# astro-turing/Integrating-diagenetic-equations-using-Python

Measured on AMD Instinct MI355X. Metric: grid-point-steps/sec (5 fields, fp64), higher is better.
Workload: dtype f64

## Files before the change

include/marl_hip.h:

```cpp
#ifndef MARL_HIP_H
#define MARL_HIP_H

#include "marl_params.h"

#ifdef __cplusplus
extern "C" {
#endif

typedef struct marl_ctx marl_ctx;

#define MARL_LAYOUT_FIELD_MAJOR 0
#define MARL_LAYOUT_TILED 1

int marl_ctx_create(const marl_params* params, int64_t n_instances, int64_t N, int device, marl_ctx** out);
int marl_ctx_set_params(marl_ctx* ctx, const marl_params* params, int64_t n_instances);

void marl_ctx_destroy(marl_ctx* ctx);
const char* marl_last_error(const marl_ctx* ctx);
int marl_set_stream(marl_ctx* ctx, void* hip_stream);
int marl_synchronize(marl_ctx* ctx);
int marl_set_option(marl_ctx* ctx, const char* name, int64_t value);
int marl_get_constants(const marl_ctx* ctx, int64_t inst, double out[19]);
int64_t marl_state_doubles(const marl_ctx* ctx, int layout);

int marl_rhs(marl_ctx* ctx, double t, const double* y, double* dydt);
int marl_rhs_dev(marl_ctx* ctx, double t, const double* y_dev, double* dydt_dev, int layout);

int marl_events(marl_ctx* ctx, const double* y, double* out);
int marl_events_dev(marl_ctx* ctx, const double* y_dev, int layout, double* out);

int marl_convert_layout_dev(marl_ctx* ctx, const double* src_dev, double* dst_dev, int src_layout, int dst_layout);

int marl_debug_math(marl_ctx* ctx, int op, const double* x_dev, double* y_dev, int64_t n, double e);

int marl_integrate_rk4(marl_ctx* ctx, double* y, double dt, int64_t nsteps);
int marl_integrate_rk4_dev(marl_ctx* ctx, double* y_dev, int layout, double dt, int64_t nsteps);
int marl_sweep_rk4_dev(marl_ctx* ctx, double* y_dev, const double* dt, int64_t nsteps);

// ... 50 lines not shown
```

integrating-diagenetic-equations-using-python_amd/_abi.py:

```python
import ctypes as C
import os

_HERE = os.path.dirname(os.path.abspath(__file__))
LIB_PATH = os.environ.get("MARL_HIP_LIBRARY") or os.path.join(_HERE, "csrc", "libmarl_hip.so")



def lab_options():
    out = []
    for item in os.environ.get("MARL_HIP_OPTIONS", "").split(","):
        if item.strip():
            name, _, value = item.partition("=")
            out.append((name.strip(), int(value)))
    return out


def library_fingerprint():
    import hashlib
    with open(LIB_PATH, "rb") as f:
        return LIB_PATH, hashlib.sha256(f.read()).hexdigest()[:16]


NFIELDS = 5
NEVENTS = 7
# ... 24 lines not shown

_P = C.c_void_p
_D = C.c_double
_I = C.c_int
_L = C.c_int64
PROTOTYPES = {
    "marl_ctx_create": (_I, [C.POINTER(MarlParams), _L, _L, _I, C.POINTER(_P)]),
    "marl_ctx_set_params": (_I, [_P, C.POINTER(MarlParams), _L]),
    "marl_ctx_destroy": (None, [_P]),
    "marl_last_error": (C.c_char_p, [_P]),
    "marl_set_stream": (_I, [_P, _P]),
    "marl_synchronize": (_I, [_P]),
    "marl_set_option": (_I, [_P, C.c_char_p, _L]),
    "marl_get_constants": (_I, [_P, _L, C.POINTER(_D)]),
    "marl_state_doubles": (_L, [_P, _I]),
    "marl_rhs": (_I, [_P, _D, _P, _P]),
    "marl_rhs_dev": (_I, [_P, _D, _P, _P, _I]),
    "marl_events": (_I, [_P, _P, _P]),
    "marl_events_dev": (_I, [_P, _P, _I, _P]),
    "marl_convert_layout_dev": (_I, [_P, _P, _P, _I, _I]),
    "marl_debug_math": (_I, [_P, _I, _P, _P, _L, _D]),
    "marl_integrate_rk4": (_I, [_P, _P, _D, _L]),
    "marl_integrate_rk4_dev": (_I, [_P, _P, _I, _D, _L]),
    "marl_sweep_rk4_dev": (_I, [_P, _P, _P, _L]),
    "marl_integrate_rk45": (_I, [_P, _P, _D, _D, _D, _D, _D, _P, _L, _P, _P, _L, _L, C.POINTER(MarlStats)]),
    "marl_integrate_rk45_dev": (_I, [_P, _P, _I, _D, _D, _D, _D, _D, _L, C.POINTER(MarlStats)]),
    "marl_sweep_rk45_dev": (_I, [_P, _P, _D, _D, _D, _D, _D, _L, C.POINTER(MarlStats)]),
    "marl_sweep_rk45_eval_dev": (_I, [_P, _P, _D, _D, _D, _D, _D, _L, _P, _L, _P, _P, C.POINTER(MarlStats)]),
    "marl_sweep_rk45_events_dev": (_I, [_P, _P, _D, _D, _D, _D, _D, _L, _P, _L, _P, _P, _P, _L, C.POINTER(MarlStats)]),
    "marl_integrate_radau": (_I, [_P, _P, _D, _D, _D, _D, _D, _P, _P, _L, _P, _P, _L, _L, C.POINTER(MarlStats)]),
# ... 53 lines not shown
```

integrating-diagenetic-equations-using-python_amd/csrc/marl_api.hip:

```cpp
#include <hip/hip_runtime.h>

#include <dlfcn.h>

#include <cmath>
#include <cstdarg>
#include <cstdio>
#include <cstring>
#include <string>
#include <vector>

#include "../../include/marl_hip.h"
#include "marl_kernels.h"
#include "marl_radau.h"
#include "marl_radau_cr.h"
#include "marl_radau_batch.h"
#include "marl_radau_wg.h"
#include "marl_bdf.h"
#include "marl_bdf_wg.h"

using namespace marl;

static_assert(MARL_NFIELDS == NF, "field count");
constexpr int64_t kChainMax = 8;
static thread_local std::string g_create_error;
// ... 48 lines not shown
    int64_t dd_max_attempts = 0;
    void* rccl_lib = nullptr;
    void* rccl_comm = nullptr;
    int (*rccl_allgather)(const void*, void*, size_t, int, void*, hipStream_t) = nullptr;
    int (*rccl_destroy)(void*) = nullptr;
    double* rd_arena = nullptr;
    size_t rd_cap = 0;
    double* rd_host = nullptr;
    double* zc_h = nullptr;
    double* zc_d = nullptr;
    bool zc_on = false;
    int64_t rk4_variant = -1, sweep_variant = -1, host_layout = LAYOUT_TILED, poll = 64;
    int64_t rk4_stream = 1;
    int64_t rk4_small = 1;
    int64_t rk4_chain = 1;
    int64_t rk4_stream_third = 1;
    double* stream_c = nullptr;
    size_t stream_c_cap = 0;
    int64_t implicit_zero_copy = 1;
    int64_t radau_fused_solve = 3;
    int64_t radau_solver = 0;
    int64_t radau_cr = -1;
    int64_t radau_cr_min_n = 2048;
    int64_t radau_cr_small = 3;
    int64_t radau_cr_small_min_n = 205;
    int64_t bdf_solve_wg = 1;
    int64_t radau_cr_tail = 1;
    int64_t radau_sweep_wg = 3;
    std::string err;
};
// ... 172 lines not shown

int marl_ctx_set_params(marl_ctx* ctx, const marl_params* params, int64_t n_instances)
{
    if (!ctx || !params) return ctx ? fail(ctx, -1, "marl_ctx_set_params: invalid argument") : -1;
    if (n_instances != ctx->batch) return fail(ctx, -1, "marl_ctx_set_params: the context holds %lld instance(s)", (long long)ctx->batch);
    if (ctx->halo > 0) return fail(ctx, -1, "marl_ctx_set_params: not for slab contexts");
    for (int64_t b = 0; b < n_instances; b++) {
        if (!(params[b].length > 0)) return fail(ctx, -1, "marl_ctx_set_params: instance %lld: length must be > 0", (long long)b);
        if ((params[b].dPhi_variable != 0) != (params[0].dPhi_variable != 0))
            return fail(ctx, -1, "marl_ctx_set_params: dPhi_variable must be the same for every instance of a sweep");
    }
    HIP_OK(ctx, hipSetDevice(ctx->device));
    HIP_OK(ctx, hipStreamSynchronize(ctx->stream));
    ctx->params.assign(params, params + n_instances);
    const int no_reuse = ctx->hconsts[0].hot.no_reuse;
    for (int64_t b = 0; b < n_instances; b++) {
        derive_consts(params[b], ctx->N, ctx->hconsts[b], &ctx->extra[4 * b]);
        ctx->hconsts[b].hot.no_reuse = no_reuse;
    }
    ctx->var_dphi = params[0].dPhi_variable != 0;
    HIP_OK(ctx, hipMemcpyAsync(ctx->dconsts, ctx->hconsts.data(), sizeof(DevConsts) * n_instances, hipMemcpyHostToDevice, ctx->stream));
    HIP_OK(ctx, hipStreamSynchronize(ctx->stream));
    return 0;
}

void marl_ctx_destroy(marl_ctx* ctx)
{
    if (!ctx) return;
    (void)hipSetDevice(ctx->device);
    (void)hipStreamSynchronize(ctx->stream);
    for (int i = 0; i < 4; i++)
        if (ctx->buf[i]) (void)hipFree(ctx->buf[i]);
    if (ctx->part) (void)hipFree(ctx->part);
    if (ctx->stream_c) (void)hipFree(ctx->stream_c);
    if (ctx->sq) (void)hipFree(ctx->sq);
    if (ctx->sq_sticky) (void)hipFree(ctx->sq_sticky);
    if (ctx->sq_host) (void)hipHostFree(ctx->sq_host);
    if (ctx->rs) (void)hipFree(ctx->rs);
    if (ctx->rs_grec) (void)hipFree(ctx->rs_grec);
    if (ctx->rs_host) (void)hipHostFree(ctx->rs_host);
    if (ctx->rec) (void)hipFree(ctx->rec);
    if (ctx->dctrl) (void)hipFree(ctx->dctrl);
    if (ctx->ddt) (void)hipFree(ctx->ddt);
    if (ctx->dconsts) (void)hipFree(ctx->dconsts);
    if (ctx->hctrl) (void)hipHostFree(ctx->hctrl);
    if (ctx->hrec) (void)hipHostFree(ctx->hrec);
    if (ctx->hdt) (void)hipHostFree(ctx->hdt);
    if (ctx->sw_teval) (void)hipFree(ctx->sw_teval);
    if (ctx->sw_ndone) (void)hipFree(ctx->sw_ndone);
// ... 60 lines not shown
    else if (n == "radau_cr_min_n") ctx->radau_cr_min_n = std::max<int64_t>(value, 4);
    else if (n == "radau_cr_small") ctx->radau_cr_small = value < 0 ? 0 : std::min<int64_t>(value, radau::CR_WG_MAX_LEVELS);
    else if (n == "radau_cr_small_min_n") ctx->radau_cr_small_min_n = std::max<int64_t>(value, 32);
    else if (n == "radau_cr_tail") ctx->radau_cr_tail = value ? 1 : 0;
    else if (n == "bdf_solve_wg") ctx->bdf_solve_wg = value ? 1 : 0;
    else if (n == "radau_fused_solve") ctx->radau_fused_solve = value < 0 ? 0 : (value > 3 ? 3 : value);
    else if (n == "radau_sweep_wg") ctx->radau_sweep_wg = value < 0 ? 0 : (value > 3 ? 3 : value);
    else if (n == "implicit_zero_copy") ctx->implicit_zero_copy = value ? 1 : 0;
    else if (n == "rk4_stream") ctx->rk4_stream = value < 0 ? 0 : (value > 2 ? 2 : value);
    else if (n == "rk45_stream") ctx->rk45_stream = value < 0 ? 0 : (value > 2 ? 2 : value);
    else if (n == "dd_stream") ctx->dd_stream = value < 0 ? 0 : (value > 2 ? 2 : value);
    else if (n == "rk45_stream_attempts") ctx->rk45_stream_attempts = value < 1 ? 1 : std::min<int64_t>(value, 1 << 20);
    else if (n == "rk4_small") ctx->rk4_small = value ? 1 : 0;
    else if (n == "rk4_chain") ctx->rk4_chain = value < 0 ? 0 : std::min<int64_t>(value, kChainMax);
    else if (n == "rk4_stream_third") ctx->rk4_stream_third = value ? 1 : 0;
    else if (n == "rk4_stream_test_raise") ctx->sq_test_raise = value != 0;
    else if (n == "rk4_stream_max_items") ctx->sq_max_items = value > 0 ? std::min<int64_t>(value, 0x7fffffff) : 0x7fffffff;
    else if (n == "no_reuse") {
        for (auto& c : ctx->hconsts) c.hot.no_reuse = value ? 1 : 0;
        HIP_OK(ctx, hipSetDevice(ctx->device));
        HIP_OK(ctx, hipStreamSynchronize(ctx->stream));
        HIP_OK(ctx, hipMemcpy(ctx->dconsts, ctx->hconsts.data(), sizeof(DevConsts) * ctx->hconsts.size(), hipMemcpyHostToDevice));
    }
    else return fail(ctx, -1, "marl_set_option: unknown option '%s'", name);
    return 0;
}

int marl_get_constants(const marl_ctx* ctx, int64_t inst, double out[19])
{
    if (!ctx || inst < 0 || inst >= ctx->batch || !out) return -1;
    const DevConsts& d = ctx->hconsts[inst];
    const HotConsts& c = d.hot;
    const double* x = &ctx->extra[4 * inst];
    const double v[19] = {x[0], c.nu1, c.nu2, c.KRat, c.dCa, c.dCO3, c.delta, c.Da, c.lambda_, x[1], x[2], c.rhorat,
                          c.presum, x[3], c.dPhi, PECLET_MIN, PECLET_MAX, (double)d.mask_lo, (double)d.mask_hi};
    memcpy(out, v, sizeof v);
    return 0;
}

int64_t marl_state_doubles(const marl_ctx* ctx, int layout) { return ctx ? state_doubles(ctx->slab.n_buf, layout) : -1; }

}

#ifndef MARL_LAB
static inline int64_t inst_stride(const marl_ctx* ctx, int layout) { return state_doubles(ctx->slab.n_buf, layout); }

static int launch_rhs(marl_ctx* ctx, const double* y, double* dydt, int layout, int64_t nstates = 0)
{
    const dim3 grid((unsigned)((ctx->slab.n_buf + 255) / 256), (unsigned)(nstates > 0 ? nstates : ctx->batch));
    const int64_t stride = inst_stride(ctx, layout);
    const int cs = nstates > 0 ? 0 : 1;
    if (ctx->var_dphi) {
        if (layout == LAYOUT_TILED)
            hipLaunchKernelGGL((rhs_kernel<LAYOUT_TILED, true>), grid, dim3(256), 0, ctx->stream, y, dydt, ctx->dconsts, ctx->slab, stride, cs);
        else
// ... 57 lines not shown
{
    constexpr int V = 256 - 8 * NSTEPS;
    const int64_t n = ctx->slab.out_hi - ctx->slab.out_lo;
    const dim3 grid((unsigned)((n + V - 1) / V));
    if (layout == LAYOUT_TILED)
        hipLaunchKernelGGL((rk4_fused_kernel<256, LAYOUT_TILED, NSTEPS, VD>), grid, dim3(256), 0, ctx->stream, yin, yout, ctx->dconsts, ctx->slab, dt);
    else
        hipLaunchKernelGGL((rk4_fused_kernel<256, LAYOUT_FIELD_MAJOR, NSTEPS, VD>), grid, dim3(256), 0, ctx->stream, yin, yout, ctx->dconsts, ctx->slab, dt);
}

constexpr int kVdRk4Depth = 4;

extern "C" int marl_small_rk4_16(int tiled, unsigned grid, hipStream_t stream, const double* yin, double* yout, const void* consts, const int64_t slab5[5],
                                 double dt);

static int launch_rk4(marl_ctx* ctx, int nsteps, const double* yin, double* yout, int layout, double dt)
{
    switch (nsteps) {
        case 1: if (ctx->var_dphi) launch_rk4_t<1, true>(ctx, yin, yout, layout, dt); else launch_rk4_t<1>(ctx, yin, yout, layout, dt); break;
        case 2: launch_rk4_t<2>(ctx, yin, yout, layout, dt); break;
        case 4: if (ctx->var_dphi) launch_rk4_t<4, true>(ctx, yin, yout, layout, dt); else launch_rk4_t<4>(ctx, yin, yout, layout, dt); break;
        case 8: launch_rk4_t<8>(ctx, yin, yout, layout, dt); break;
        case 16: {
            const int64_t n = ctx->slab.out_hi - ctx->slab.out_lo, V = 256 - 8 * 16, tiles = (n + V - 1) / V;
            if (!ctx->cus) {
                hipDeviceProp_t prop;
                HIP_OK(ctx, hipGetDeviceProperties(&prop, ctx->device));
                ctx->cus = prop.multiProcessorCount;
            }
            if (ctx->rk4_small && tiles <= 2 * (int64_t)ctx->cus) {
                const int64_t slab5[5] = {ctx->slab.n_buf, ctx->slab.goff, ctx->slab.ld, ctx->slab.out_lo, ctx->slab.out_hi};
                const int e = marl_small_rk4_16(layout == LAYOUT_TILED, (unsigned)tiles, ctx->stream, yin, yout, ctx->dconsts, slab5, dt);
// ... 99 lines not shown
    while (levels > 0) {
        const int64_t cap = (ctx->sq_max_items / tiles) & ~(int64_t)1;
        const int64_t lv = std::min<int64_t>(levels, std::max<int64_t>(cap, 2));
        const unsigned blocks = (unsigned)std::min<int64_t>(lv * tiles, (4 * 256 / MARL_LAB_STREAM_BLK) * (int64_t)ctx->cus);
        double* c = nullptr;
        if (ctx->rk4_stream_third && levels == lv && (lv & 1) && lv >= 3) {
            const size_t need = (size_t)state_doubles(ctx->slab.n_buf, layout);
            if (ctx->stream_c_cap < need) {
                if (ctx->stream_c) HIP_OK(ctx, hipFree(ctx->stream_c));
                ctx->stream_c = nullptr; ctx->stream_c_cap = 0;
                HIP_OK(ctx, hipMalloc((void**)&ctx->stream_c, need * sizeof(double)));
                ctx->stream_c_cap = need;
            }
            c = ctx->stream_c;
        }
        if (K >= 2) {
            if (layout == LAYOUT_TILED) launch_chain_t<LAYOUT_TILED>(ctx, a, b, dt, (unsigned)lv, shape, blocks, c);
            else launch_chain_t<LAYOUT_FIELD_MAJOR>(ctx, a, b, dt, (unsigned)lv, shape, blocks, c);
        } else switch (per) {
            case 1: if (ctx->var_dphi) launch_stream_t<1, true>(ctx, a, b, layout, dt, (unsigned)lv, (unsigned)tiles, blocks, c);
                    else launch_stream_t<1>(ctx, a, b, layout, dt, (unsigned)lv, (unsigned)tiles, blocks, c);
                    break;
            case 2: launch_stream_t<2>(ctx, a, b, layout, dt, (unsigned)lv, (unsigned)tiles, blocks, c); break;
            case 4: if (ctx->var_dphi) launch_stream_t<4, true>(ctx, a, b, layout, dt, (unsigned)lv, (unsigned)tiles, blocks, c);
                    else launch_stream_t<4>(ctx, a, b, layout, dt, (unsigned)lv, (unsigned)tiles, blocks, c);
                    break;
            case 8: launch_stream_t<8>(ctx, a, b, layout, dt, (unsigned)lv, (unsigned)tiles, blocks, c); break;
            case 16: launch_stream_t<16>(ctx, a, b, layout, dt, (unsigned)lv, (unsigned)tiles, blocks, c); break;
            default: return fail(ctx, -1, "rk4 stream: %d steps per level not instantiated", per);
        }
// ... 2187 lines not shown
```

integrating-diagenetic-equations-using-python_amd/csrc/marl_kernels.h:

```cpp
#pragma once
#include <type_traits>

#include "marl_math.h"
#include "marl_brent.h"

namespace marl {

enum : int { LAYOUT_FIELD_MAJOR = 0, LAYOUT_TILED = 1 };

template <int LAYOUT>
__device__ __forceinline__ int64_t at(int f, int64_t i, int64_t ld)
{
    if constexpr (LAYOUT == LAYOUT_FIELD_MAJOR)
        return (int64_t)f * ld + i;
    else
        return (i >> 6) * (int64_t)(NF * 64) + f * 64 + (i & 63);
}

struct Slab {
    int64_t n_buf;
    int64_t goff;
    int64_t ld;
    int64_t out_lo;
    int64_t out_hi;
// ... 5 lines not shown
__device__ __forceinline__ double mon_min(double a, double b) { return FINITE ? __builtin_fmin(a, b) : nanmin(a, b); }
template <bool FINITE = false>
__device__ __forceinline__ double mon_max(double a, double b) { return FINITE ? __builtin_fmax(a, b) : nanmax(a, b); }


#ifdef MARL_LAB_PHASE_CLOCK
__device__ unsigned long long marl_lab_phase[8];
#define MARL_PHASE_MARK(k) do { const unsigned long long t_ = __builtin_amdgcn_s_memtime(); ph_acc[k] += t_ - ph_last; ph_last = t_; } while (0)
#else
#define MARL_PHASE_MARK(k) do { } while (0)
#endif

#define MARL_ONCE _Pragma("unroll") for (int once_ = 0; once_ < 1; once_++)
#define MARL_FIELDS _Pragma("unroll") for (int f = 0; f < NF; f++)

template <int BLK, bool REUSE = true, bool VD = false, int SEAM = 0>
struct StencilBlock {
    static constexpr int EDGE_DOUBLES = 2 * NF * BLK;
    static constexpr bool CACHE_LDS = PC_LDS_SLOTS > 0;
    static constexpr bool CACHE = REUSE && (EDGE_DOUBLES + TABLE_DOUBLES + PC_LDS_SLOTS * BLK) * 8 <= 60 * 1024;
    static constexpr int CACHE_DOUBLES = CACHE ? PC_LDS_SLOTS * BLK : 0;
    static constexpr int LDS_DOUBLES = EDGE_DOUBLES + TABLE_DOUBLES + CACHE_DOUBLES;

    double* lds;
    Tables T;
    HotConsts K;
    const DevConsts* C;
    int tid;
    int parity;
    unsigned masks;
    static constexpr bool EDGE_ONCE = CACHE;
    unsigned edge_cells;
    __device__ __forceinline__ bool edge_wave() const
    {
        if constexpr (EDGE_ONCE) return edge_cells & 1u;
        else return __builtin_amdgcn_ballot_w64(is_edge() != 0) != 0;
    }
    __device__ __forceinline__ unsigned is_first() const { return masks & 1u; }
    __device__ __forceinline__ unsigned is_last() const { return (masks >> 8) & 1u; }
    __device__ __forceinline__ unsigned in_zone() const { return (masks >> 16) & 1u; }
    __device__ __forceinline__ unsigned is_edge() const { return masks & 0x101u; }
    PointCache<(CACHE && CACHE_LDS) ? BLK : 0> cache;
    bool reuse_live = false;
    static constexpr int SEAM_STRIDE = 16, SEAM_READS = 0x10000, SEAM_WAVE0 = 0x20000, SEAM_WAVEW = 0x40000;
    static_assert(SEAM < BLK, "the recording lane is a lane of the window");
    double* seam = nullptr;
// ... 36 lines not shown
#pragma unroll
        for (int f = 0; f < NF; f++) e[f * BLK + tid] = ys[f];
        if constexpr (SEAM > 0) {
            if (seam_pos & SEAM_WAVEW) {
                int tw = tid;
                asm volatile("" : "+v"(tw));
                if (tw == SEAM) {
                    double* rec = seam + (seam_pos & 0xffff);
#pragma unroll
                    for (int f = 0; f < NF; f++) rec[f] = ys[f];
                }
            }
        }
        MARL_PHASE_MARK(0);
        PointLocal pl;
        MARL_ONCE point_local<CACHE ? MODE : TR_PLAIN, (CACHE && CACHE_LDS) ? BLK : 0, VD>(ys, in_zone(), K, C, T, pl, aux, cache, reuse_live);
        MARL_PHASE_MARK(1);
        __syncthreads();
        MARL_PHASE_MARK(2);
        const int tl = tid > 0 ? tid - 1 : 0;
        const int tr = tid < BLK - 1 ? tid + 1 : BLK - 1;
        double left[NF], right[NF];
#pragma unroll
        for (int f = 0; f < NF; f++) left[f] = e[f * BLK + tl];
        if constexpr (SEAM > 0) {
            if ((seam_pos & (SEAM_WAVE0 | SEAM_READS)) == (SEAM_WAVE0 | SEAM_READS)) {
                int t0 = tid;
                asm volatile("" : "+v"(t0));
                if (t0 == 0) {
                    const double* prev = seam + ((seam_pos & 0xffff) ^ 8);
#pragma unroll
// ... 283 lines not shown

#ifndef MARL_LAB_RK4_WAVES_MIN
#define MARL_LAB_RK4_WAVES_MIN 4
#define MARL_LAB_RK4_WAVES_MAX 8
#endif
template <int BLK, int LAYOUT, int NSTEPS, bool VD = false>
__global__ void __launch_bounds__(BLK) __attribute__((amdgpu_waves_per_eu(MARL_LAB_RK4_WAVES_MIN, MARL_LAB_RK4_WAVES_MAX))) rk4_fused_kernel(const double* __restrict__ yin, double* __restrict__ yout,
                                                        const DevConsts* __restrict__ consts, Slab S, double dt)
{
#ifdef MARL_LAB_CLOCK
    const unsigned long long lab_t0 = __builtin_amdgcn_s_memtime(), lab_r0 = __builtin_amdgcn_s_memrealtime();
#endif
    constexpr int H = 4 * NSTEPS;
    constexpr int V = BLK - 2 * H;
    static_assert(V > 0, "window too small for the fused halo");
    using SB = StencilBlock<BLK, true, VD>;
    __shared__ double lds[SB::LDS_DOUBLES];
    const DevConsts& C = consts[0];

    const int64_t w0 = S.out_lo + (int64_t)blockIdx.x * V - H;
    const int64_t l = w0 + (int64_t)threadIdx.x;
    double y[NF];
    load_cells<LAYOUT>(yin, l, S, C, y);
    SB sb(lds, l + S.goff, consts);
    rk4_advance<NSTEPS>(sb, y, dt);

    const int wi = threadIdx.x;
    MARL_ONCE if (wi >= H && wi < BLK - H && l >= S.out_lo && l < S.out_hi) {
#pragma unroll
        for (int f = 0; f < NF; f++) yout[at<LAYOUT>(f, l, S.ld)] = y[f];
    }
#ifdef MARL_LAB_PHASE_CLOCK
    sb.phase_flush();
#endif
#ifdef MARL_LAB_CLOCK
    if (threadIdx.x == 0 && blockIdx.x < 16384) {
        marl_lab_clock[3 * blockIdx.x] = __builtin_amdgcn_s_memtime() - lab_t0;
        marl_lab_clock[3 * blockIdx.x + 1] = __builtin_amdgcn_s_memrealtime() - lab_r0;
        marl_lab_clock[3 * blockIdx.x + 2] = lab_r0;
    }
#endif
}

constexpr unsigned STREAM_SPIN_LIMIT = 1u << 19;

template <int BLK, int LAYOUT, int NSTEPS, bool VD = false>
__global__ void __launch_bounds__(BLK) __attribute__((amdgpu_waves_per_eu(4, 8)))
rk4_stream_kernel(double* bufA, double* bufB, const DevConsts* __restrict__ consts, Slab S, double dt, unsigned levels, unsigned tiles,
                  unsigned* queue, unsigned* done, unsigned* sticky, unsigned item_base, unsigned level_base, double* bufC = nullptr)
{
    constexpr int H = 4 * NSTEPS;
    constexpr int V = BLK - 2 * H;
    using SB = StencilBlock<BLK, true, VD>;
    __shared__ double lds[SB::LDS_DOUBLES];
    __shared__ unsigned s_item, s_abort;
    const DevConsts& C = consts[0];
    SB sb(lds, 0, consts);
    const unsigned total = levels * tiles;

#ifdef MARL_LAB_BROKEN_STREAM_LATCH
    if (threadIdx.x == 0) {
        s_item = __hip_atomic_fetch_add(&queue[0], 1u, __ATOMIC_RELAXED, __HIP_MEMORY_SCOPE_AGENT) - item_base;
        s_abort = 0;
    }
    while (true) {
        __syncthreads();
#else
    while (true) {
// ... 25 lines not shown
            }
            __syncthreads();
            if (s_abort) break;
        }
        const double* src = bufC ? (level == 0 ? bufA : ((level & 1u) ? bufB : bufC)) : ((level & 1u) ? bufB : bufA);
        double* dst = bufC ? (level + 1 == levels ? bufA : ((level & 1u) ? bufC : bufB)) : ((level & 1u) ? bufA : bufB);
        const int64_t l = S.out_lo + (int64_t)tile * V - H + threadIdx.x;
        const bool in = l >= 0 && l < S.n_buf;
        double y[NF];
#pragma unroll
        for (int f = 0; f < NF; f++)
            y[f] = in ? __hip_atomic_load(src + at<LAYOUT>(f, l, S.ld), __ATOMIC_RELAXED, __HIP_MEMORY_SCOPE_AGENT) : C.bc[f];
        sb.set_window(l + S.goff);
        sb.reuse_live = false;
        rk4_advance<NSTEPS>(sb, y, dt);
        if ((int)threadIdx.x >= H && (int)threadIdx.x < BLK - H && l >= S.out_lo && l < S.out_hi) {
#pragma unroll
            for (int f = 0; f < NF; f++) __hip_atomic_store(dst + at<LAYOUT>(f, l, S.ld), y[f], __ATOMIC_RELAXED, __HIP_MEMORY_SCOPE_AGENT);
        }
        __atomic_signal_fence(__ATOMIC_SEQ_CST);
        __builtin_amdgcn_s_waitcnt(0);
        __atomic_signal_fence(__ATOMIC_SEQ_CST);
        __syncthreads();
        if (threadIdx.x == 0) {
            __hip_atomic_store(&done[tile], level_base + level + 1u, __ATOMIC_RELAXED, __HIP_MEMORY_SCOPE_AGENT);
#ifdef MARL_LAB_BROKEN_STREAM_LATCH
            s_item = __hip_atomic_fetch_add(&queue[0], 1u, __ATOMIC_RELAXED, __HIP_MEMORY_SCOPE_AGENT) - item_base;
            s_abort = 0;
#endif
        }
    }
}

template <int BLK, int LAYOUT, int NSTEPS>
__global__ void __launch_bounds__(BLK) __attribute__((amdgpu_waves_per_eu(4, 8)))
rk4_chain_kernel(double* bufA, double* bufB, const DevConsts* __restrict__ consts, Slab S, double dt, unsigned levels, unsigned items,
                 unsigned* queue, unsigned* done, unsigned* sticky, unsigned item_base, unsigned level_base, double* bufC,
                 unsigned K, unsigned nsub_last, int64_t bound)
{
    constexpr int H = 4 * NSTEPS;
    constexpr int V = BLK - 2 * H;
    constexpr int W = BLK - H;
    static_assert(V > 0, "window too small for the fused halo");
    using SB = StencilBlock<BLK, true, false, BLK - H - 1>;
    __shared__ double lds[SB::LDS_DOUBLES];
    __shared__ double seam[H * SB::SEAM_STRIDE];
    __shared__ unsigned s_item, s_abort;
    const DevConsts& C = consts[0];
    SB sb(lds, 0, consts);
    sb.seam = seam;
    const unsigned total = levels * items;
    const unsigned chains = items - 1;

    while (true) {
        __syncthreads();
        if (threadIdx.x == 0) {
            s_item = __hip_atomic_fetch_add(&queue[0], 1u, __ATOMIC_RELAXED, __HIP_MEMORY_SCOPE_AGENT) - item_base;
            s_abort = 0;
        }
// ... 1414 lines not shown
```

integrating-diagenetic-equations-using-python_amd/csrc/marl_math.h:

```cpp
#pragma once
#include <hip/hip_runtime.h>
#include <stddef.h>
#include <stdint.h>

#include "marl_tables.h"

namespace marl {

constexpr int NF = 5;

struct HotConsts {
    double inv_dx, inv_dx2;
    double presum, rhorat;
    double KRat, nu1, nu2;
    double lambda_, Da, delta;
    double dCa, dCO3, dPhi;
    double pe_cCa, pe_cCO3, pe_Phi;
    double m1, m2, n1, n2;
    double hdx;
    double pe_smax;
    double Dal;
    double Da_nu1, Dal_nu2;
    double rr10;
    double dPhi_dx2;
    double auxcon;
    int32_t fv;
    int32_t generic_p0;
    int32_t var_dphi;
    int32_t no_reuse;
};

struct DevConsts {
    HotConsts hot;
    double p0_m1, p0_m2, p0_n1, p0_n2;
    double bc[NF];
    int64_t N;
    int64_t mask_lo, mask_hi;
    int64_t reserved;
};

constexpr double PECLET_MIN = 1e-2, PECLET_MAX = 1.0 / PECLET_MIN;
constexpr double FV_SERIES_MAX = 0.5;

__device__ __forceinline__ double pin_uniform(double v)
{
    asm volatile("" : "+s"(v));
    return v;
}

__device__ __forceinline__ HotConsts load_hot(const DevConsts* __restrict__ c)
{
    HotConsts k = c->hot;
    double* f = reinterpret_cast<double*>(&k);
#pragma unroll
// ... 117 lines not shown
enum : int { PC_INVPHI, PC_INVOM, PC_INVDEN, PC_IB, PC_E, PC_TC, PC_SLOTS };
constexpr int PC_FIRST_LDS = PC_SLOTS - (MARL_CACHE_LDS_SLOTS < PC_SLOTS ? MARL_CACHE_LDS_SLOTS : PC_SLOTS);
constexpr int PC_LDS_SLOTS = PC_SLOTS - PC_FIRST_LDS;

template <int STRIDE>
struct PointCache {
    static constexpr int FIRST_LDS = STRIDE > 0 ? PC_FIRST_LDS : PC_SLOTS;
    double Phi, O2, cPhi, nib;
    double* s;
    double v[FIRST_LDS > 0 ? FIRST_LDS : 1];
    bool fv_quiet;
    __device__ __forceinline__ double get(int j) const { return j < FIRST_LDS ? v[j] : s[(j - FIRST_LDS) * STRIDE]; }
    __device__ __forceinline__ void set(int j, double x) { if (j < FIRST_LDS) v[j] = x; else s[(j - FIRST_LDS) * STRIDE] = x; }
};

template <int MODE>
__device__ __forceinline__ double ten_operand()
{
    if constexpr (MODE == TR_PLAIN) return 10.0;
    else return pin_uniform(10.0);
}

struct PointLocal {
    double Ux, R0, R1;
    double W, invPhi, G2, G3;
    double h1x, h2f;
    double Q4, DaR;
    double Wd;
    bool upw, fv_active;
    bool fv_solutes;
};

#pragma clang diagnostic push
#pragma clang diagnostic ignored "-Wsometimes-uninitialized"
template <int MODE, int STRIDE, bool VD = false, bool LEGACY = false>
__device__ __forceinline__ void point_local(const double (&uc)[NF], bool in_mask, const HotConsts& K, const DevConsts* __restrict__ C,
                                            const Tables& T, PointLocal& pl, PointAux& aux, PointCache<STRIDE>& pc, bool& live)
{
    static_assert(!LEGACY || MODE == TR_PLAIN, "the legacy operation order is the stand-alone RHS's (no transcendental cache)");
#ifdef MARL_ABLATE_CORE
    aux.U = aux.W = 0.0;
    return;
#endif
    const double CA = uc[0], CC = uc[1], c = uc[2], o = uc[3], Phi = uc[4];
    const double omPhi = 1.0 - Phi;
    const double O2 = c * o;

    double den, invPhi, invom, invden, ex, tC, tA;
    bool fv_check = K.fv != 0;
    bool reuse = false;
    if constexpr (MODE == TR_FILL) live = false;
    if ((MODE == TR_REUSE || MODE == TR_AUTO) && live) {
        const double d = Phi - pc.Phi, dO = O2 - pc.O2;
        const double v = dO * pc.nib;
        const double big = __builtin_fma(fabs(d), pc.cPhi, fabs(v));
        reuse = __builtin_amdgcn_ballot_w64(!(big < REUSE_LIMIT)) == 0;
        live = reuse;
        if (reuse) {
            const bool tiny = __builtin_amdgcn_ballot_w64(!(big < REUSE_TINY)) == 0;
            const double invPhi0 = pc.get(PC_INVPHI), invom0 = pc.get(PC_INVOM), invden0 = pc.get(PC_INVDEN), ib0 = pc.get(PC_IB);
            const double e0 = pc.get(PC_E), tC0 = pc.get(PC_TC);
            const double x = d * invPhi0, y = d * invom0, u = dO * ib0;
            double l1p, ip, w, gy;
            double da;
            if (__builtin_expect(tiny, 1)) {
                l1p = x * __builtin_fma(x, -0.5, 1.0);
                const double t10 = invPhi0 * __builtin_fma(-x, x, x);
                ip = invPhi0 - t10;
                da = 10.0 * t10;
                w = v * __builtin_fma(u, -0.5, 1.0);
                gy = __builtin_fma(y, 1.0 + y, 1.0);
            } else {
                l1p = x * __builtin_fma(x, __builtin_fma(x, 1.0 / 3, -0.5), 1.0);
// ... 52 lines not shown
        if (K.generic_p0) {
            asm volatile("");
            const double y1 = C->p0_n1, y2 = C->p0_n2, nu2 = C->hot.nu2;
            const double pcw = (O2 == 1.0) ? (over ? y1 : y2) : pwC;
            tC = (LEGACY ? 1.0 : K.Dal) * (over ? pcw - nu2 * y2 : y1 - nu2 * pcw);
        }
        if constexpr (MODE == TR_FILL || MODE == TR_AUTO) {
            const double ib = (K.generic_p0 | K.no_reuse) ? __builtin_nan("") : rcp_nr(O2 - 1.0);
            pc.Phi = Phi; pc.O2 = O2; pc.nib = nsel * ib;
            pc.cPhi = fmax(fmax(fabs(invPhi), fabs(invom)), fmax(12.0 * (invPhi * invPhi), 2.2 * fabs(invPhi * invden)));
            pc.set(PC_INVPHI, invPhi); pc.set(PC_INVOM, invom); pc.set(PC_INVDEN, invden); pc.set(PC_E, ex);
            pc.set(PC_IB, ib); pc.set(PC_TC, tC);
            live = true;
        }
    }
    {
        const double O3 = O2 * K.KRat;
        const bool under = O3 < 1.0;
        tA = O3 - O3;
        if (!under || in_mask) {
#ifdef MARL_ABLATE_POWA
            const double pwA = fabs(O3 - 1.0) * (under ? K.m2 : K.m1);
#else
            const double pwA = pow_sat(fabs(O3 - 1.0), under ? K.m2 : K.m1, T);
#endif
            tA = (LEGACY ? (under ? 1.0 : -K.nu1) : (under ? K.Da : -K.Da_nu1)) * pwA;
        }
        if (K.generic_p0) {
            asm volatile("");
            const double z1 = C->p0_m1, z2 = C->p0_m2, nu1 = C->hot.nu1;
            const double mask = in_mask ? 1.0 : 0.0;
            const double pa = (O3 == 1.0) ? (under ? z2 : z1) : ((!under || in_mask) ? fast_exp((under ? K.m2 : K.m1) * fast_log(fabs(O3 - 1.0), T), T) : 0.0);
            tA = (LEGACY ? 1.0 : K.Da) * (under ? pa * mask - nu1 * z1 : z2 * mask - nu1 * pa);
        }
    }
    const double rF = LEGACY ? K.rhorat * (1.0 - ex) : __builtin_fma(-K.rhorat, ex, K.rhorat);
    const double t2 = rF * (Phi * Phi);
    const double W = K.presum - t2;
    const double U = __builtin_fma(t2 * Phi, invom, K.presum);
    aux.U = U;
    aux.W = W;
    double wpe = fabs(W) * K.pe_Phi;
    if constexpr (VD) {
        const double dPhi = K.auxcon * ((1.0 - ex) * (Phi * Phi)) * (Phi * invom);
        wpe = fabs(W) * (K.pe_Phi * (K.dPhi * rcp_nr(dPhi)));
    }

    const double DA = LEGACY ? K.Da * (CA * tA) : CA * tA;
// ... 106 lines not shown
    double diffusion;
    if constexpr (VD) {
        diffusion = __builtin_fma(dPhi_cell() * K.inv_dx2, p_d, pl.DaR);
    } else {
        diffusion = __builtin_fma(K.dPhi_dx2, p_d, pl.DaR);
    }
    r[4] = __builtin_fma(-pg, pl.Q4, diffusion);
}

template <int MODE, int STRIDE, bool VD = false>
__device__ __forceinline__ void rhs_point(const double (&uc)[NF], const double (&um)[NF], const double (&up)[NF],
                                          bool in_mask, const HotConsts& K, const DevConsts* __restrict__ C,
                                          const Tables& T, double (&r)[NF], PointAux& aux, PointCache<STRIDE>& pc, bool& live)
{
    PointLocal pl;
    point_local<MODE, STRIDE, VD, true>(uc, in_mask, K, C, T, pl, aux, pc, live);
    point_rates<VD, false, true>(uc, um, up, K, T, pl, r);
}


}
```

integrating-diagenetic-equations-using-python_amd/csrc/marl_rk4_small.hip:

```cpp
#define marl marl_small
#define MARL_CACHE_LDS_SLOTS 0
#define MARL_LAB_RK4_WAVES_MIN 1
#define MARL_LAB_RK4_WAVES_MAX 2
#include "marl_kernels.h"
#undef marl

extern "C" __attribute__((visibility("hidden"))) int marl_small_rk4_16(int tiled, unsigned grid, hipStream_t stream, const double* yin, double* yout,
                                                                       const void* consts, const int64_t slab5[5], double dt)
{
    using namespace marl_small;
    const Slab S{slab5[0], slab5[1], slab5[2], slab5[3], slab5[4]};
    const DevConsts* c = static_cast<const DevConsts*>(consts);
    if (tiled)
        hipLaunchKernelGGL((rk4_fused_kernel<256, LAYOUT_TILED, 16>), dim3(grid), dim3(256), 0, stream, yin, yout, c, S, dt);
    else
        hipLaunchKernelGGL((rk4_fused_kernel<256, LAYOUT_FIELD_MAJOR, 16>), dim3(grid), dim3(256), 0, stream, yin, yout, c, S, dt);
    return (int)hipGetLastError();
}
```

Baseline: 52.38 billion.

## Cache aragonite rate term per point in global memory and reuse via Taylor update

Adds a per-point global scratch buffer (pointed to from DevConsts) that stores the aragonite reaction term and a reciprocal derivative factor when it is first computed in a fused RK4 block. On later stages where the saturation ratio changes only slightly and the whole wave stays on one side of saturation, the kernel updates the cached value with a second-order expansion instead of calling pow. This is meant to remove expensive fp64 transcendental work from the fused fixed-step kernels. The cost is extra global reads and writes of 16 bytes per point, extra host synchronisation and copies when the buffer grows, and a small approximation error that is bounded by the reuse threshold.

```diff
diff --git a/include/marl_hip.h b/include/marl_hip.h
--- a/include/marl_hip.h
+++ b/include/marl_hip.h
@@ -22,6 +22,7 @@
 int marl_set_option(marl_ctx* ctx, const char* name, int64_t value);
 int marl_get_constants(const marl_ctx* ctx, int64_t inst, double out[19]);
 int64_t marl_state_doubles(const marl_ctx* ctx, int layout);
+void marl_consts_layout(int64_t out[4]);
 
 int marl_rhs(marl_ctx* ctx, double t, const double* y, double* dydt);
 int marl_rhs_dev(marl_ctx* ctx, double t, const double* y_dev, double* dydt_dev, int layout);
diff --git a/integrating-diagenetic-equations-using-python_amd/_abi.py b/integrating-diagenetic-equations-using-python_amd/_abi.py
--- a/integrating-diagenetic-equations-using-python_amd/_abi.py
+++ b/integrating-diagenetic-equations-using-python_amd/_abi.py
@@ -62,6 +62,7 @@
     "marl_set_option": (_I, [_P, C.c_char_p, _L]),
     "marl_get_constants": (_I, [_P, _L, C.POINTER(_D)]),
     "marl_state_doubles": (_L, [_P, _I]),
+    "marl_consts_layout": (None, [C.POINTER(_L)]),
     "marl_rhs": (_I, [_P, _D, _P, _P]),
     "marl_rhs_dev": (_I, [_P, _D, _P, _P, _I]),
     "marl_events": (_I, [_P, _P, _P]),
diff --git a/integrating-diagenetic-equations-using-python_amd/csrc/marl_api.hip b/integrating-diagenetic-equations-using-python_amd/csrc/marl_api.hip
--- a/integrating-diagenetic-equations-using-python_amd/csrc/marl_api.hip
+++ b/integrating-diagenetic-equations-using-python_amd/csrc/marl_api.hip
@@ -86,6 +86,9 @@
     int64_t rk4_stream = 1;
     int64_t rk4_small = 1;
     int64_t rk4_chain = 1;
+    double* ara = nullptr;
+    int64_t ara_cap = 0;
+    int64_t ara_reuse = 1;
     int64_t rk4_stream_third = 1;
     double* stream_c = nullptr;
     size_t stream_c_cap = 0;
@@ -288,9 +291,11 @@
     HIP_OK(ctx, hipStreamSynchronize(ctx->stream));
     ctx->params.assign(params, params + n_instances);
     const int no_reuse = ctx->hconsts[0].hot.no_reuse;
+    double* const ara = ctx->hconsts[0].ara;
     for (int64_t b = 0; b < n_instances; b++) {
         derive_consts(params[b], ctx->N, ctx->hconsts[b], &ctx->extra[4 * b]);
         ctx->hconsts[b].hot.no_reuse = no_reuse;
+        ctx->hconsts[b].ara = ara;
     }
     ctx->var_dphi = params[0].dPhi_variable != 0;
     HIP_OK(ctx, hipMemcpyAsync(ctx->dconsts, ctx->hconsts.data(), sizeof(DevConsts) * n_instances, hipMemcpyHostToDevice, ctx->stream));
@@ -307,6 +312,7 @@
         if (ctx->buf[i]) (void)hipFree(ctx->buf[i]);
     if (ctx->part) (void)hipFree(ctx->part);
     if (ctx->stream_c) (void)hipFree(ctx->stream_c);
+    if (ctx->ara) (void)hipFree(ctx->ara);
     if (ctx->sq) (void)hipFree(ctx->sq);
     if (ctx->sq_sticky) (void)hipFree(ctx->sq_sticky);
     if (ctx->sq_host) (void)hipHostFree(ctx->sq_host);
@@ -397,6 +403,7 @@
     else if (n == "rk4_small") ctx->rk4_small = value ? 1 : 0;
     else if (n == "rk4_chain") ctx->rk4_chain = value < 0 ? 0 : std::min<int64_t>(value, kChainMax);
     else if (n == "rk4_stream_third") ctx->rk4_stream_third = value ? 1 : 0;
+    else if (n == "ara_reuse") ctx->ara_reuse = value ? 1 : 0;
     else if (n == "rk4_stream_test_raise") ctx->sq_test_raise = value != 0;
     else if (n == "rk4_stream_max_items") ctx->sq_max_items = value > 0 ? std::min<int64_t>(value, 0x7fffffff) : 0x7fffffff;
     else if (n == "no_reuse") {
@@ -422,6 +429,15 @@
 }
 
 int64_t marl_state_doubles(const marl_ctx* ctx, int layout) { return ctx ? state_doubles(ctx->slab.n_buf, layout) : -1; }
+
+extern "C" __attribute__((visibility("hidden"))) void marl_small_consts_layout(int64_t out[2]);
+
+void marl_consts_layout(int64_t out[4])
+{
+    out[0] = (int64_t)sizeof(DevConsts);
+    out[1] = (int64_t)offsetof(DevConsts, ara);
+    marl_small_consts_layout(out + 2);
+}
 
 }
 
@@ -509,8 +525,35 @@
 extern "C" int marl_small_rk4_16(int tiled, unsigned grid, hipStream_t stream, const double* yin, double* yout, const void* consts, const int64_t slab5[5],
                                  double dt);
 
+constexpr int64_t kAraMaxBlocks = (int64_t)1 << 18;
+static int ensure_ara(marl_ctx* ctx, int64_t blocks)
+{
+    double* want = nullptr;
+    if (ctx->ara_reuse && !ctx->var_dphi && blocks <= kAraMaxBlocks) {
+        if (ctx->ara_cap < blocks) {
+            HIP_OK(ctx, hipStreamSynchronize(ctx->stream));
+            if (ctx->ara) HIP_OK(ctx, hipFree(ctx->ara));
+            ctx->ara = nullptr;
+            ctx->ara_cap = 0;
+            HIP_OK(ctx, hipMalloc((void**)&ctx->ara, (size_t)blocks * 256 * 2 * sizeof(double)));
+            ctx->ara_cap = blocks;
+        }
+        want = ctx->ara;
+    }
+    if (ctx->hconsts[0].ara != want) {
+        for (auto& c : ctx->hconsts) c.ara = want;
+        HIP_OK(ctx, hipStreamSynchronize(ctx->stream));
+        HIP_OK(ctx, hipMemcpy(ctx->dconsts, ctx->hconsts.data(), sizeof(DevConsts) * ctx->hconsts.size(), hipMemcpyHostToDevice));
+    }
+    return 0;
+}
+
 static int launch_rk4(marl_ctx* ctx, int nsteps, const double* yin, double* yout, int layout, double dt)
 {
+    if (nsteps >= 1 && nsteps <= 16) {
+        const int64_t n = ctx->slab.out_hi - ctx->slab.out_lo, V = 256 - 8 * nsteps;
+        if (int rc = ensure_ara(ctx, (n + V - 1) / V)) return rc;
+    }
     switch (nsteps) {
         case 1: if (ctx->var_dphi) launch_rk4_t<1, true>(ctx, yin, yout, layout, dt); else launch_rk4_t<1>(ctx, yin, yout, layout, dt); break;
         case 2: launch_rk4_t<2>(ctx, yin, yout, layout, dt); break;
@@ -640,6 +683,7 @@
             }
             c = ctx->stream_c;
         }
+        if (int rc = ensure_ara(ctx, blocks)) return rc;
         if (K >= 2) {
             if (layout == LAYOUT_TILED) launch_chain_t<LAYOUT_TILED>(ctx, a, b, dt, (unsigned)lv, shape, blocks, c);
             else launch_chain_t<LAYOUT_FIELD_MAJOR>(ctx, a, b, dt, (unsigned)lv, shape, blocks, c);
diff --git a/integrating-diagenetic-equations-using-python_amd/csrc/marl_kernels.h b/integrating-diagenetic-equations-using-python_amd/csrc/marl_kernels.h
--- a/integrating-diagenetic-equations-using-python_amd/csrc/marl_kernels.h
+++ b/integrating-diagenetic-equations-using-python_amd/csrc/marl_kernels.h
@@ -43,7 +43,10 @@
 #define MARL_ONCE _Pragma("unroll") for (int once_ = 0; once_ < 1; once_++)
 #define MARL_FIELDS _Pragma("unroll") for (int f = 0; f < NF; f++)
 
-template <int BLK, bool REUSE = true, bool VD = false, int SEAM = 0>
+#ifndef MARL_ARA_REUSE
+#define MARL_ARA_REUSE 1
+#endif
+template <int BLK, bool REUSE = true, bool VD = false, int SEAM = 0, bool ARA = false>
 struct StencilBlock {
     static constexpr int EDGE_DOUBLES = 2 * NF * BLK;
     static constexpr bool CACHE_LDS = PC_LDS_SLOTS > 0;
@@ -59,6 +62,8 @@
     int parity;
     unsigned masks;
     static constexpr bool EDGE_ONCE = CACHE;
+    static constexpr bool ARA_CENTRE = ARA;
+    static_assert(!ARA || (CACHE && !VD), "the aragonite centre comes with the transcendental cache");
     unsigned edge_cells;
     __device__ __forceinline__ bool edge_wave() const
     {
@@ -125,7 +130,8 @@
         }
         MARL_PHASE_MARK(0);
         PointLocal pl;
-        MARL_ONCE point_local<CACHE ? MODE : TR_PLAIN, (CACHE && CACHE_LDS) ? BLK : 0, VD>(ys, in_zone(), K, C, T, pl, aux, cache, reuse_live);
+        MARL_ONCE point_local<CACHE ? MODE : TR_PLAIN, (CACHE && CACHE_LDS) ? BLK : 0, VD, false, ARA>(ys, in_zone(), K, C, T, pl, aux, cache, reuse_live, edge_cells,
+                                                                                                     ARA ? blockIdx.x * BLK : 0u, (unsigned)tid);
         MARL_PHASE_MARK(1);
         __syncthreads();
         MARL_PHASE_MARK(2);
@@ -439,7 +445,7 @@
     constexpr int H = 4 * NSTEPS;
     constexpr int V = BLK - 2 * H;
     static_assert(V > 0, "window too small for the fused halo");
-    using SB = StencilBlock<BLK, true, VD>;
+    using SB = StencilBlock<BLK, true, VD, 0, MARL_ARA_REUSE && !VD>;
     __shared__ double lds[SB::LDS_DOUBLES];
     const DevConsts& C = consts[0];
 
@@ -450,10 +456,20 @@
     SB sb(lds, l + S.goff, consts);
     rk4_advance<NSTEPS>(sb, y, dt);
 
+    if constexpr (SB::ARA_CENTRE) {
+        int ts = threadIdx.x;
+        asm volatile("" : "+v"(ts));
+        const int64_t ls = w0 + ts;
+        MARL_ONCE if (ts >= H && ts < BLK - H && ls >= S.out_lo && ls < S.out_hi) {
+#pragma unroll
+            for (int f = 0; f < NF; f++) yout[at<LAYOUT>(f, ls, S.ld)] = y[f];
+        }
+    } else {
     const int wi = threadIdx.x;
     MARL_ONCE if (wi >= H && wi < BLK - H && l >= S.out_lo && l < S.out_hi) {
 #pragma unroll
         for (int f = 0; f < NF; f++) yout[at<LAYOUT>(f, l, S.ld)] = y[f];
+    }
     }
 #ifdef MARL_LAB_PHASE_CLOCK
     sb.phase_flush();
@@ -476,7 +492,7 @@
 {
     constexpr int H = 4 * NSTEPS;
     constexpr int V = BLK - 2 * H;
-    using SB = StencilBlock<BLK, true, VD>;
+    using SB = StencilBlock<BLK, true, VD, 0, MARL_ARA_REUSE && !VD>;
     __shared__ double lds[SB::LDS_DOUBLES];
     __shared__ unsigned s_item, s_abort;
     const DevConsts& C = consts[0];
@@ -532,6 +548,15 @@
         sb.set_window(l + S.goff);
         sb.reuse_live = false;
         rk4_advance<NSTEPS>(sb, y, dt);
+        if constexpr (SB::ARA_CENTRE) {
+            int ts = threadIdx.x;
+            asm volatile("" : "+v"(ts));
+            const int64_t ls = S.out_lo + (int64_t)tile * V - H + ts;
+            if (ts >= H && ts < BLK - H && ls >= S.out_lo && ls < S.out_hi) {
+#pragma unroll
+                for (int f = 0; f < NF; f++) __hip_atomic_store(dst + at<LAYOUT>(f, ls, S.ld), y[f], __ATOMIC_RELAXED, __HIP_MEMORY_SCOPE_AGENT);
+            }
+        } else
         if ((int)threadIdx.x >= H && (int)threadIdx.x < BLK - H && l >= S.out_lo && l < S.out_hi) {
 #pragma unroll
             for (int f = 0; f < NF; f++) __hip_atomic_store(dst + at<LAYOUT>(f, l, S.ld), y[f], __ATOMIC_RELAXED, __HIP_MEMORY_SCOPE_AGENT);
@@ -560,7 +585,7 @@
     constexpr int V = BLK - 2 * H;
     constexpr int W = BLK - H;
     static_assert(V > 0, "window too small for the fused halo");
-    using SB = StencilBlock<BLK, true, false, BLK - H - 1>;
+    using SB = StencilBlock<BLK, true, false, BLK - H - 1, MARL_ARA_REUSE != 0>;
     __shared__ double lds[SB::LDS_DOUBLES];
     __shared__ double seam[H * SB::SEAM_STRIDE];
     __shared__ unsigned s_item, s_abort;
diff --git a/integrating-diagenetic-equations-using-python_amd/csrc/marl_math.h b/integrating-diagenetic-equations-using-python_amd/csrc/marl_math.h
--- a/integrating-diagenetic-equations-using-python_amd/csrc/marl_math.h
+++ b/integrating-diagenetic-equations-using-python_amd/csrc/marl_math.h
@@ -36,8 +36,10 @@
     double bc[NF];
     int64_t N;
     int64_t mask_lo, mask_hi;
-    int64_t reserved;
+    double* ara;
 };
+static_assert(sizeof(HotConsts) == 30 * 8 && offsetof(DevConsts, ara) == sizeof(HotConsts) + 12 * 8 && sizeof(DevConsts) == sizeof(HotConsts) + 13 * 8,
+              "DevConsts layout");
 
 constexpr double PECLET_MIN = 1e-2, PECLET_MAX = 1.0 / PECLET_MIN;
 constexpr double FV_SERIES_MAX = 0.5;
@@ -185,6 +187,15 @@
     __device__ __forceinline__ void set(int j, double x) { if (j < FIRST_LDS) v[j] = x; else s[(j - FIRST_LDS) * STRIDE] = x; }
 };
 
+constexpr unsigned ARA_LIVE = 2u, ARA_UNDER = 4u;
+typedef double ara_pair_t __attribute__((ext_vector_type(2)));
+typedef __attribute__((address_space(1))) ara_pair_t* ara_ptr_t;
+__device__ __forceinline__ ara_ptr_t ara_slot(const DevConsts* __restrict__ C, unsigned abase, unsigned atid)
+{
+    asm volatile("" : "+v"(atid));
+    return (ara_ptr_t)((__attribute__((address_space(1))) char*)C->ara + (abase + atid) * 16u);
+}
+
 template <int MODE>
 __device__ __forceinline__ double ten_operand()
 {
@@ -204,11 +215,13 @@
 
 #pragma clang diagnostic push
 #pragma clang diagnostic ignored "-Wsometimes-uninitialized"
-template <int MODE, int STRIDE, bool VD = false, bool LEGACY = false>
+template <int MODE, int STRIDE, bool VD = false, bool LEGACY = false, bool ARA = false>
 __device__ __forceinline__ void point_local(const double (&uc)[NF], bool in_mask, const HotConsts& K, const DevConsts* __restrict__ C,
-                                            const Tables& T, PointLocal& pl, PointAux& aux, PointCache<STRIDE>& pc, bool& live)
+                                            const Tables& T, PointLocal& pl, PointAux& aux, PointCache<STRIDE>& pc, bool& live,
+                                            unsigned& aflags, unsigned abase, unsigned atid)
 {
     static_assert(!LEGACY || MODE == TR_PLAIN, "the legacy operation order is the stand-alone RHS's (no transcendental cache)");
+    static_assert(!ARA || (MODE != TR_PLAIN && !VD), "the aragonite centre belongs to the cached fixed-step kernels");
 #ifdef MARL_ABLATE_CORE
     aux.U = aux.W = 0.0;
     return;
@@ -218,6 +231,7 @@
     const double O2 = c * o;
 
     double den, invPhi, invom, invden, ex, tC, tA;
+    ara_pair_t ara0;
     bool fv_check = K.fv != 0;
     bool reuse = false;
     if constexpr (MODE == TR_FILL) live = false;
@@ -228,6 +242,9 @@
         reuse = __builtin_amdgcn_ballot_w64(!(big < REUSE_LIMIT)) == 0;
         live = reuse;
         if (reuse) {
+            if constexpr (ARA) {
+                if (aflags & ARA_LIVE) ara0 = *ara_slot(C, abase, atid);
+            }
             const bool tiny = __builtin_amdgcn_ballot_w64(!(big < REUSE_TINY)) == 0;
             const double invPhi0 = pc.get(PC_INVPHI), invom0 = pc.get(PC_INVOM), invden0 = pc.get(PC_INVDEN), ib0 = pc.get(PC_IB);
             const double e0 = pc.get(PC_E), tC0 = pc.get(PC_TC);
@@ -310,11 +327,33 @@
             live = true;
         }
     }
-    {
+    bool ara_reused = false;
+    if constexpr (ARA) {
+        if (reuse && (aflags & ARA_LIVE)) {
+            asm volatile("");
+            const double uA = (O2 - pc.O2) * ara0.y;
+            const double mu = ((aflags & ARA_UNDER) ? K.m2 : K.m1) * uA;
+            ara_reused = __builtin_amdgcn_ballot_w64(!(fmax(fabs(uA), fabs(mu)) < REUSE_TINY)) == 0;
+            if (ara_reused) {
+                const double wA = mu * __builtin_fma(uA, -0.5, 1.0);
+                tA = ara0.x * __builtin_fma(wA, __builtin_fma(wA, 0.5, 1.0), 1.0);
+            } else {
+                aflags &= ~ARA_LIVE;
+            }
+        }
+    }
+    if (!ara_reused) {
         const double O3 = O2 * K.KRat;
         const bool under = O3 < 1.0;
         tA = O3 - O3;
+        unsigned long long takes = 0, takes_under = 0;
         if (!under || in_mask) {
+            if constexpr (ARA && (MODE == TR_FILL || MODE == TR_AUTO)) {
+                double o3 = O3;
+                asm volatile("" : "+v"(o3));
+                takes = __builtin_amdgcn_ballot_w64(true);
+                takes_under = __builtin_amdgcn_ballot_w64(o3 < 1.0);
+            }
 #ifdef MARL_ABLATE_POWA
             const double pwA = fabs(O3 - 1.0) * (under ? K.m2 : K.m1);
 #else
@@ -328,6 +367,21 @@
             const double mask = in_mask ? 1.0 : 0.0;
             const double pa = (O3 == 1.0) ? (under ? z2 : z1) : ((!under || in_mask) ? fast_exp((under ? K.m2 : K.m1) * fast_log(fabs(O3 - 1.0), T), T) : 0.0);
             tA = (LEGACY ? 1.0 : K.Da) * (under ? pa * mask - nu1 * z1 : z2 * mask - nu1 * pa);
+        }
+        if constexpr (ARA && (MODE == TR_FILL || MODE == TR_AUTO)) {
+            if (!reuse) {
+                aflags &= ~(ARA_LIVE | ARA_UNDER);
+                if (takes != 0 && (takes_under == 0 || takes_under == takes) && !(K.generic_p0 | K.no_reuse)) {
+                    asm volatile("");
+                    if (C->ara) {
+                        ara_pair_t a;
+                        a.x = tA;
+                        a.y = rcp_nr(O2 - rcp_nr(K.KRat));
+                        *ara_slot(C, abase, atid) = a;
+                        aflags |= ARA_LIVE | (takes_under ? ARA_UNDER : 0u);
+                    }
+                }
+            }
         }
     }
     const double rF = LEGACY ? K.rhorat * (1.0 - ex) : __builtin_fma(-K.rhorat, ex, K.rhorat);
@@ -464,7 +518,8 @@
                                           const Tables& T, double (&r)[NF], PointAux& aux, PointCache<STRIDE>& pc, bool& live)
 {
     PointLocal pl;
-    point_local<MODE, STRIDE, VD, true>(uc, in_mask, K, C, T, pl, aux, pc, live);
+    unsigned no_ara = 0;
+    point_local<MODE, STRIDE, VD, true>(uc, in_mask, K, C, T, pl, aux, pc, live, no_ara, 0u, 0u);
     point_rates<VD, false, true>(uc, um, up, K, T, pl, r);
 }
 
diff --git a/integrating-diagenetic-equations-using-python_amd/csrc/marl_rk4_small.hip b/integrating-diagenetic-equations-using-python_amd/csrc/marl_rk4_small.hip
--- a/integrating-diagenetic-equations-using-python_amd/csrc/marl_rk4_small.hip
+++ b/integrating-diagenetic-equations-using-python_amd/csrc/marl_rk4_small.hip
@@ -2,6 +2,7 @@
 #define MARL_CACHE_LDS_SLOTS 0
 #define MARL_LAB_RK4_WAVES_MIN 1
 #define MARL_LAB_RK4_WAVES_MAX 2
+#define MARL_ARA_REUSE 0
 #include "marl_kernels.h"
 #undef marl
 
@@ -17,3 +18,9 @@
         hipLaunchKernelGGL((rk4_fused_kernel<256, LAYOUT_FIELD_MAJOR, 16>), dim3(grid), dim3(256), 0, stream, yin, yout, c, S, dt);
     return (int)hipGetLastError();
 }
+
+extern "C" __attribute__((visibility("hidden"))) void marl_small_consts_layout(int64_t out[2])
+{
+    out[0] = (int64_t)sizeof(marl_small::DevConsts);
+    out[1] = (int64_t)offsetof(marl_small::DevConsts, ara);
+}
```

Measured after the change: 52.05 billion. No clear change (-0.6%).
